# WestlyPark/StyleRenderer

Hardware: AMD Instinct MI355X
Metric: generator fwd+bwd images/sec at 256^2 (higher is better)
Workload: dtype f32

## Files before the change

### include/stylerenderer_amd.h

```cpp
#ifndef STYLERENDERER_AMD_H_
#define STYLERENDERER_AMD_H_

#include <stddef.h>
#include <stdint.h>

#ifdef __cplusplus
extern "C" {
#endif

typedef void* sr_stream_t;

#define SR_OK 0
#define SR_EINVAL (-1)
#define SR_ERANGE (-2)

const char* sr_error_string(int code);
int sr_abi_version(void);

int sr_fused_bias_act(float* y, const float* x, const float* b, const float* ref, int act, int grad,
                      float alpha, float scale, int64_t size_x, int64_t step_b, int64_t size_b,
                      int use_bias, int use_ref, sr_stream_t stream);

int64_t sr_fused_act_bwd_scratch_floats(int64_t n, int64_t c, int64_t inner);
int sr_fused_act_bwd(float* gx, float* gb, const float* gy, const float* out, float alpha,
// ... 258 lines not shown
int sr_conv2d_generic_dgrad(float* dx, const float* g, const float* w, int64_t B, int64_t C, int64_t N, int64_t IH,
                            int64_t IW, int64_t OH, int64_t OW, int kh, int kw, int sy, int sx, int py, int px,
                            sr_stream_t stream);
int sr_conv2d_generic_wgrad(float* dw, const float* x, const float* g, int64_t B, int64_t C, int64_t N, int64_t IH,
                            int64_t IW, int64_t OH, int64_t OW, int kh, int kw, int sy, int sx, int py, int px,
                            sr_stream_t stream);
int sr_conv2d_mfma_ex(float* out, const float* in, const float* wt, const float* iscale,
                      const float* oscale, const float* obias, int64_t B, int64_t C, int64_t N,
                      int64_t wt_ld, int64_t IH, int64_t IW, int64_t OH, int64_t OW, int ksize,
                      int stride, int pad, int transposed, int flags, float* scratch, sr_stream_t stream);
int sr_conv1x1_add_supported(int64_t B, int64_t C, int64_t N, int64_t wt_ld, int64_t P, const float* in, const float* wt,
                             const float* out, const float* addend);
int sr_conv1x1_add(float* out, const float* in, const float* wt, const float* oscale, const float* addend, int64_t B,
                   int64_t C, int64_t N, int64_t wt_ld, int64_t P, sr_stream_t stream);
int sr_conv2d_nba_ex(float* out, const float* in, const float* wt, const float* iscale, const float* oscale,
                     const float* noise, const float* noise_w, const float* abias, float alpha, float gain,
                     int64_t B, int64_t C, int64_t N, int64_t wt_ld, int64_t H, int64_t W, int64_t noise_bstride,
                     int flags, float* scratch, sr_stream_t stream);

int64_t sr_conv2d_wgrad_scratch_floats(int64_t B, int64_t C, int64_t N, int64_t IH, int64_t IW,
                                       int64_t OH, int64_t OW, int ksize, int stride, int pad,
                                       int transposed);
int sr_conv2d_wgrad_mfma(float* dwt, const float* x, const float* gy, const float* xscale,
                         const float* gscale, int64_t B, int64_t C, int64_t N, int64_t IH,
                         int64_t IW, int64_t OH, int64_t OW, int ksize, int stride, int pad,
                         int transposed, float* scratch, sr_stream_t stream);
#define SR_WGRAD_PATH_INVALID (-1)
#define SR_WGRAD_PATH_DIRECT 0
#define SR_WGRAD_PATH_SMALL3 1
#define SR_WGRAD_PATH_WINO 2
#define SR_WGRAD_PATH_BF16_1X1 3
#define SR_WGRAD_PATH_BF16_S2 4
#define SR_WGRAD_PATH_S2_DMA 5
int sr_conv2d_wgrad_path(int64_t B, int64_t C, int64_t N, int64_t IH, int64_t IW, int64_t OH, int64_t OW, int ksize,
                         int stride, int pad, int transposed, const float* x, const float* gy);

int sr_signal_bump(uint32_t* counter, sr_stream_t stream);
int sr_signal_set(uint32_t* word, const uint32_t* epoch, sr_stream_t stream);
int sr_signal_wait(const uint32_t* counter, uint32_t at_least, sr_stream_t stream);
int sr_signal_wait_timeout(const uint32_t* counter, uint32_t at_least, uint64_t timeout_us, int32_t* status_host,
                           int32_t code, sr_stream_t stream);
int sr_signal_wait_poison(const uint32_t* counter, uint32_t at_least, uint64_t timeout_us, int32_t* status_host,
                          int32_t code, float* poison, sr_stream_t stream);
int sr_signal_set_host(uint32_t* word_host, const uint32_t* epoch, sr_stream_t stream);

int sr_graph_replace_memset_nodes(void* hip_graph, int* replaced);
int sr_graph_node_count(void* graph, int* kernel_nodes, int* all_nodes);

int64_t sr_lpips_layer_scratch_floats(int64_t b, int64_t hw);
int sr_lpips_layer_fwd(float* d, const float* f0, const float* t, const float* lin, int64_t b, int64_t c, int64_t hw,
                       int64_t t_bstride, float eps, float* scratch, sr_stream_t stream);
int sr_lpips_layer_bwd(float* gf, const float* gd, const float* f0, const float* t, const float* lin, int64_t b,
                       int64_t c, int64_t hw, int64_t t_bstride, float eps, sr_stream_t stream);
int sr_ppl_endpoints(float* out, const float* a, const float* b, int64_t in_stride, const float* t, int64_t npairs,
                     int64_t d, int mode, int n_ends, float eps, sr_stream_t stream);
int sr_ppl_prep(float* out, const float* img, const float* shift, const float* scale, int64_t n, int64_t h, int64_t w,
                int64_t y0, int64_t x0, int64_t ch, int64_t cw, int64_t oh, int64_t ow, sr_stream_t stream);
int64_t sr_lpips_pair_scratch_floats(int64_t npairs, int64_t n_layers, const int64_t* hw);
int sr_lpips_pair(float* d, const float* const* f, const float* const* lin, const int64_t* c, const int64_t* hw,
                  int64_t n_layers, int64_t npairs, float div, float* scratch, sr_stream_t stream);
int sr_incep_conv(const float* in, const float* wt, const float* bias, int64_t B, int64_t C, int64_t H, int64_t W,
                  int64_t M, int kh, int kw, int stride, int ph, int pw, int nseg, float* const* seg_out,
                  const int64_t* seg_m0, const int64_t* seg_coff, const int64_t* seg_ctot, sr_stream_t stream);
int sr_incep_pool(float* out, const float* in, int64_t B, int64_t C, int64_t H, int64_t W, int mode, int64_t coff,
                  int64_t ctot, sr_stream_t stream);
int sr_incep_gap(float* out, const float* in, int64_t planes, int64_t hw, sr_stream_t stream);
int sr_fstats_update(double* sum, double* gram, double* shift, const float* f, int64_t n, int64_t d, int first,
                     sr_stream_t stream);
// ... 84 lines not shown
```

### stylerenderer_amd/_lib.py

```python
import ctypes
import os

_HERE = os.path.dirname(os.path.abspath(__file__))
LIB_PATH = os.environ.get("STYLERENDERER_AMD_LIB") or os.path.join(_HERE, "libstylerenderer_hip.so")

_i = ctypes.c_int
_l = ctypes.c_int64
_f = ctypes.c_float
_d = ctypes.c_double
_p = ctypes.c_void_p

SIGNATURES = {
    "sr_error_string": (ctypes.c_char_p, [_i]),
    "sr_abi_version": (_i, []),
    "sr_fused_bias_act": (_i, [_p, _p, _p, _p, _i, _i, _f, _f, _l, _l, _l, _i, _i, _p]),
    "sr_fused_act_bwd_scratch_floats": (_l, [_l, _l, _l]),
    "sr_fused_act_bwd": (_i, [_p, _p, _p, _p, _f, _f, _l, _l, _l, _p, _p]),
    "sr_noise_bias_act": (_i, [_p] * 6 + [_f, _f] + [_l] * 4 + [_p]),
    "sr_noise_bias_act_bwd_scratch_floats": (_l, [_l, _l, _l]),
    "sr_noise_bias_act_bwd": (_i, [_p] * 6 + [_f, _f] + [_l] * 4 + [_p, _p]),
    "sr_noise_bias_act_bwd_dot_scratch_floats": (_l, [_l, _l, _l]),
    "sr_noise_bias_act_bwd_dot": (_i, [_p] * 9 + [_f, _f] + [_l] * 4 + [_p, _p]),
    "sr_conv2d_nba": (_i, [_p] * 8 + [_f, _f] + [_l] * 7 + [_p, _p]),
    "sr_conv2d_nba_ex": (_i, [_p] * 8 + [_f, _f] + [_l] * 7 + [_i, _p, _p]),
# ... 55 lines not shown
    "sr_ada_apply": (_i, [_p] * 3 + [_l] * 3 + [_i, _p]),
    "sr_ada_apply_grad": (_i, [_p] * 3 + [_l] * 3 + [_p]),
    "sr_ada_update": (_i, [_p, _p, _d, _d, _p]),
    "sr_upfirdn2d": (_i, [_p, _p, _p, _l] + [_i] * 14 + [_p]),
    "sr_upsample2_add": (_i, [_p] * 4 + [_l] + [_i] * 6 + [_p]),
    "sr_blur_noise_bias_act": (_i, [_p] * 6 + [_f, _f, _l, _l] + [_i] * 6 + [_l, _p]),
    "sr_conv2d_generic": (_i, [_p] * 4 + [_l] * 7 + [_i] * 6 + [_p]),
    "sr_conv2d_generic_dgrad": (_i, [_p] * 3 + [_l] * 7 + [_i] * 6 + [_p]),
    "sr_conv2d_generic_wgrad": (_i, [_p] * 3 + [_l] * 7 + [_i] * 6 + [_p]),
    "sr_blur_nba_bwd_scratch_floats": (_l, [_l, _l, _i, _i]),
    "sr_blur_nba_bwd": (_i, [_p] * 10 + [_f, _f, _l, _l] + [_i] * 5 + [_l, _p, _p]),
    "sr_rasterize_scratch_bytes": (_l, [_l, _l, _l, _l, _i]),
    "sr_rasterize_forward_f32": (_i, [_l] * 5 + [_i] * 3 + [_p] * 5 + [_f, _p, _l, _p, _p, _p, _p, _p]),
    "sr_rasterize_levels_supported": (_i, [_i, _l, _l, _p, _p]),
    "sr_rasterize_forward_levels_f32": (_i, [_i, _l, _l, _l, _p, _p, _i, _i, _i, _p, _p, _f, _p, _l, _p, _p, _p, _p, _p]),
    "sr_rasterize_grad_levels_f32": (_i, [_i, _l, _l, _l, _p, _p, _i, _i, _p, _p, _l] + [_p] * 6 + [_l, _l] + [_p] * 3 + [_f, _p, _p]),
    "sr_rasterize_forward_f64": (_i, [_l] * 5 + [_i] * 3 + [_p] * 5 + [_d, _p, _l, _p, _p, _p, _p, _p]),
    "sr_rasterize_grad_scratch_bytes": (_l, [_l, _l, _l, _i]),
    "sr_rasterize_forward_cpu_f32": (_i, [_l] * 5 + [_i] * 3 + [_p] * 5 + [_f]),
    "sr_rasterize_forward_cpu_f64": (_i, [_l] * 5 + [_i] * 3 + [_p] * 5 + [_d]),
    "sr_rasterize_backward_cpu_f32": (_i, [_l] * 4 + [_i] + [_p] * 3 + [_f]),
    "sr_rasterize_backward_cpu_f64": (_i, [_l] * 4 + [_i] + [_p] * 3 + [_d]),
    "sr_rasterize_backward_f32": (_i, [_l] * 4 + [_i] * 2 + [_p] * 3 + [_f, _p]),
    "sr_rasterize_backward_f64": (_i, [_l] * 4 + [_i] * 2 + [_p] * 3 + [_d, _p]),
    "sr_rasterize_grad_f32": (_i, [_l] * 5 + [_i] * 2 + [_p, _p, _l] + [_p] * 6 + [_l, _l, _p, _p, _p, _f, _p, _p]),
    "sr_conv2d_wgrad_scratch_floats": (_l, [_l] * 7 + [_i] * 4),
    "sr_conv2d_wgrad_mfma": (_i, [_p] * 5 + [_l] * 7 + [_i] * 4 + [_p, _p]),
    "sr_conv2d_scratch_floats": (_l, [_l] * 7 + [_i] * 4),
    "sr_conv2d_mfma": (_i, [_p] * 6 + [_l] * 8 + [_i] * 4 + [_p, _p]),
    "sr_conv2d_uses_winograd": (_i, [_l] * 5 + [_p, _p]),
    "sr_conv2d_path": (_i, [_l] * 7 + [_i] * 4 + [_p, _p, _p, _l, _i]),
    "sr_conv2d_path_floats": (_l, [_l] * 7 + [_i] * 4 + [_p, _p, _p, _l, _i]),
    "sr_conv2d_wgrad_path": (_i, [_l] * 7 + [_i] * 4 + [_p, _p]),
    "sr_conv2d_mfma_ex": (_i, [_p] * 6 + [_l] * 8 + [_i] * 5 + [_p, _p]),
    "sr_conv1x1_add_supported": (_i, [_l] * 5 + [_p] * 4),
    "sr_conv1x1_add": (_i, [_p] * 5 + [_l] * 5 + [_p]),
    "sr_rasterize_grad_f64": (_i, [_l] * 5 + [_i] * 2 + [_p, _p, _l] + [_p] * 6 + [_l, _l, _p, _p, _p, _d, _p, _p]),
    "sr_pose_fwd": (_i, [_p, _p, _p, _p]),
    "sr_pose_bwd": (_i, [_p, _p, _p, _p, _p]),
    "sr_pose_batch_fwd": (_i, [_p, _p, _p, _l, _p]),
    "sr_affine3_fwd": (_i, [_p, _p, _p, _p, _l, _l, _l, _p]),
    "sr_affine3_bwd": (_i, [_p, _p, _p, _p, _l, _l, _l, _p]),
    "sr_morph_fwd": (_i, [_p] * 9 + [_f, _l, _l, _l, _p]),
    "sr_vertex_normals_bwd_f32": (_i, [_p] * 11 + [_l, _l, _l, _f, _p]),
    "sr_morph_gcoeff_scratch_floats": (_l, [_l, _l, _l]),
    "sr_morph_gcoeff": (_i, [_p] * 6 + [_f, _p, _l, _l, _l, _p]),
    "sr_morph_pose_bwd": (_i, [_p] * 5 + [_l, _p]),
    "sr_skin_joints_fwd": (_i, [_p] * 11 + [_f] + [_l] * 4 + [_p]),
    "sr_skin_fwd": (_i, [_p] * 7 + [_l] * 4 + [_p]),
    "sr_skin_bwd_scratch_floats": (_l, [_l, _l, _l]),
    "sr_skin_bwd": (_i, [_p] * 7 + [_l] * 3 + [_p]),
    "sr_skin_joints_bwd": (_i, [_p] * 11 + [_f, _p] + [_l] * 5 + [_p]),
    "sr_blend_z_floats": (_l, [_l, _l, _l]),
    "sr_blend_head": (_i, [_p] * 6 + [_f] + [_l] * 3 + [_p]),
    "sr_blend_fwd": (_i, [_p] * 8 + [_l] * 4 + [_p]),
    "sr_blend_gz": (_i, [_p] * 3 + [_l] * 4 + [_p]),
    "sr_blend_tail": (_i, [_p] * 5 + [_f, _p] + [_l] * 3 + [_p]),
    "sr_resample_u8_scratch_bytes": (_l, [_l] * 6 + [ctypes.POINTER(ctypes.c_int32)] + [_l] * 4),
    "sr_resample_u8": (_i, [_p, _p] + [_l] * 6 + [_p, _p, ctypes.POINTER(ctypes.c_int32), _l] * 2 + [_l] * 4
                       + [_i, _i, _p, _p]),
    "sr_warp_affine_u8": (_i, [_p, _p, _p] + [_l] * 7 + [_i, _i, _i, _p]),
    "sr_landmark_loss_fwd": (_i, [_p] * 8 + [_l] * 5 + [_f, _f, _p]),
    "sr_landmark_loss_bwd": (_i, [_p, _p, _p, _l, _p, _p, _p] + [_l] * 5 + [_i, _p]),
    "sr_landmark_dyn_fwd": (_i, [_p] * 15 + [_l] * 6 + [_i, _f, _f, _l, _l, _f, _f, _p]),
    "sr_landmark_dyn_bwd": (_i, [_p, _p, _p, _l] + [_p] * 7 + [_l] * 6 + [_i, _p]),
    "sr_region_fill": (_i, [_p, _p, _p] + [_l] * 6 + [_p]),
    "sr_region_grow": (_i, [_p, _p, _l, _l, _l, _i, _p]),
    "sr_region_blend_fwd": (_i, [_p] * 6 + [_l] * 4 + [_f] + [_l] * 4 + [_p]),
    "sr_region_blend_bwd": (_i, [_p] * 3 + [_l] * 4 + [_p]),
    "sr_texture_bake": (_i, [_p] * 9 + [_l] * 10 + [_f, _f, _f, _p]),
    "sr_texture_pad": (_i, [_p] * 4 + [_l] * 4 + [_p]),
    "sr_texture_merge": (_i, [_p] * 5 + [_l] * 4 + [_i, _p]),
    "sr_share_rows": (_i, [_p] + [_l] * 3 + [_p]),
    "sr_camera_fwd": (_i, [_p] * 5 + [_l, _l, _p]),
    "sr_camera_bwd": (_i, [_p] * 6 + [_l, _l, _p]),
    "sr_signal_bump": (_i, [_p, _p]),
    "sr_signal_wait": (_i, [_p, ctypes.c_uint32, _p]),
    "sr_signal_set": (_i, [_p, _p, _p]),
    "sr_signal_set_host": (_i, [_p, _p, _p]),
    "sr_signal_wait_timeout": (_i, [_p, ctypes.c_uint32, ctypes.c_uint64, _p, _i, _p]),
    "sr_signal_wait_poison": (_i, [_p, ctypes.c_uint32, ctypes.c_uint64, _p, _i, _p, _p]),
    "sr_graph_replace_memset_nodes": (_i, [_p, ctypes.POINTER(_i)]),
    "sr_graph_node_count": (_i, [_p, ctypes.POINTER(_i), ctypes.POINTER(_i)]),
}

(CONV_PATH_DIRECT, CONV_PATH_WINO, CONV_PATH_S2_BF16, CONV_PATH_S2_WINO, CONV_PATH_GEMM1X1, CONV_PATH_CONVT_TAPS,
 CONV_PATH_CONVT_BF16, CONV_PATH_CONVT_FUSED_KS, CONV_PATH_CONVT_FUSED) = range(9)
CONV_PATH_STRIPS = 0x100
(WGRAD_PATH_DIRECT, WGRAD_PATH_SMALL3, WGRAD_PATH_WINO, WGRAD_PATH_BF16_1X1, WGRAD_PATH_BF16_S2,
 WGRAD_PATH_S2_DMA) = range(6)

_lib = None


class NativeLibraryError(RuntimeError):
    pass


def lib():
    global _lib
    if _lib is not None:
        return _lib
    if not os.path.isfile(LIB_PATH):
        raise NativeLibraryError(
            "stylerenderer_amd: %s not found. Build it with `python -c 'import __graft_entry__ as g; "
            "g.build()'` (hipcc --offload-arch=gfx950). There is no CPU/PyTorch fallback for device "
            "tensors." % LIB_PATH)
    try:
        handle = ctypes.CDLL(LIB_PATH)
    except OSError as e:
        raise NativeLibraryError("stylerenderer_amd: cannot load %s: %s" % (LIB_PATH, e))
    for name, (res, args) in SIGNATURES.items():
        try:
            fn = getattr(handle, name)
        except AttributeError:
            raise NativeLibraryError("stylerenderer_amd: %s does not export %s" % (LIB_PATH, name))
        fn.restype = res
        fn.argtypes = args
    _lib = handle
    return _lib


def check(rc, what=""):
# ... 17 lines not shown
```

### stylerenderer_amd/build.py

```python
import os
import subprocess
import sys

HERE = os.path.dirname(os.path.abspath(__file__))
CSRC = os.path.join(HERE, "csrc")
LIB = os.path.join(HERE, "libstylerenderer_hip.so")
OBJ = os.path.join(HERE, "csrc", "_obj")

ARCH = "gfx950"
COMMON = ["--offload-arch=" + ARCH, "-O3", "-std=c++17", "-fPIC", "-Wno-unused-result",
          "-fhip-fp32-correctly-rounded-divide-sqrt"]
EXACT = ["-ffp-contract=off"]
NOSLP = ["-fno-slp-vectorize"]

SOURCES = [
    ("capi.hip", EXACT),
    ("fused_bias_act.hip", EXACT),
    ("upfirdn2d.hip", EXACT + NOSLP),
    ("rasterize.hip", EXACT),
    ("fused_elem.hip", EXACT),
    ("weight_prep.hip", EXACT),
    ("style_linear.hip", EXACT),
    ("bank_mm.hip", EXACT),
    ("mesh.hip", EXACT),
    ("landmark.hip", EXACT),
    ("region.hip", EXACT),
    ("texture.hip", EXACT),
    ("share.hip", EXACT),
    ("camera.hip", EXACT),
    ("morph.hip", []),
    ("skin.hip", []),
    ("blend.hip", []),
    ("lpips.hip", EXACT),
    ("ppl.hip", EXACT),
    ("augment.hip", EXACT),
    ("resample.hip", EXACT),
    ("warp.hip", EXACT),
    ("conv_mfma.hip", []),
    ("conv_wino.hip", []),
    ("conv_wgrad_wino.hip", []),
    ("conv_wgrad_mfma.hip", []),
    ("conv_wgrad_bf16x3.hip", []),
    ("conv_s2_bf16x3.hip", []),
    ("conv_s2_wino.hip", []),
    ("conv_generic.hip", []),
    ("conv1x1_gemm.hip", []),
    ("inception.hip", []),
]


def _hipcc():
    for c in (os.environ.get("HIPCC"), "/opt/rocm/bin/hipcc", "hipcc"):
        if c and (os.path.isabs(c) and os.path.exists(c) or not os.path.isabs(c)):
            return c
    return "hipcc"


def _deps(src):
    deps = [src, os.path.join(CSRC, "common.h"),
            os.path.join(HERE, "..", "include", "stylerenderer_amd.h"), os.path.abspath(__file__)]
    deps += [os.path.join(CSRC, f) for f in os.listdir(CSRC) if f.endswith(".h")]
    return max(os.path.getmtime(d) for d in deps if os.path.exists(d))


def build_library(force=False, verbose=False):
    os.makedirs(OBJ, exist_ok=True)
    hipcc = _hipcc()
    objs, rebuilt = [], False
    procs = []
    for name, extra in SOURCES:
        src = os.path.join(CSRC, name)
        obj = os.path.join(OBJ, name.replace(".hip", ".o"))
        objs.append(obj)
        if force or not os.path.exists(obj) or os.path.getmtime(obj) < _deps(src):
            cmd = [hipcc] + COMMON + extra + ["-c", src, "-o", obj]
# ... 22 lines not shown
```

### stylerenderer_amd/csrc/conv_wgrad_mfma.hip

```cpp
#include "common.h"
#include "conv_wgrad_bf16x3.h"
#include "conv_wino.h"

#include <algorithm>
#include <cstdlib>

namespace {

typedef float f32x16 __attribute__((ext_vector_type(16)));
typedef const void __attribute__((address_space(1)))* gptr_t;
typedef void __attribute__((address_space(3)))* lptr_t;

__device__ __attribute__((aligned(16))) const float g_wzero_line[4] = {0.f, 0.f, 0.f, 0.f};
__device__ __attribute__((aligned(16))) const float g_wones_line[4] = {1.f, 1.f, 1.f, 1.f};

struct WgradParams {
    const float* U;
    const float* V;
    const float* uscale;
    const float* vscale;
    float* partial;
    int B, CU, CV;
    int UH, UW;
    int GH, GW;
    int dy0, dx0;
    int tiles_x, tiles_y, tiles_b;
    int tiles_u, tiles_v;
    int ks, patches_per_slice;
    int UP, VP;
};

template <int IS, int TY, int TX, int PW, int PH, int PB, int UT, int VT, int NG>
struct WG {
    static constexpr int NWAVE = 4 * NG, THREADS = 256 * NG;
// ... 395 lines not shown
    int pw, ph, pb, ut, vt;
    int tiles_x, tiles_y, tiles_b, tiles_u, tiles_v, ks, pps;
};

Plan make_plan(int is, int B, int CU, int CV, int GH, int GW) {
    Plan pl;
    if (is == 1) {
        if (GW > 16) { pl.pw = 32; pl.ph = 2; pl.pb = 1; }
        else if (GW > 8) { pl.pw = 16; pl.ph = 4; pl.pb = 1; }
        else if (GW > 4) { pl.pw = 8; pl.ph = 8; pl.pb = 1; }
        else { pl.pw = 4; pl.ph = 4; pl.pb = 4; }
        pl.ut = 64; pl.vt = 64;
    } else {
        if (GW > 8) { pl.pw = 16; pl.ph = 4; pl.pb = 1; }
        else { pl.pw = 8; pl.ph = 8; pl.pb = 1; }
        pl.ut = 32; pl.vt = 128;
    }
    pl.tiles_x = (GW + pl.pw - 1) / pl.pw;
    pl.tiles_y = (GH + pl.ph - 1) / pl.ph;
    pl.tiles_b = (B + pl.pb - 1) / pl.pb;
    pl.tiles_u = (CU + pl.ut - 1) / pl.ut;
    pl.tiles_v = (CV + pl.vt - 1) / pl.vt;
    const int npatch = pl.tiles_x * pl.tiles_y * pl.tiles_b;
    const int tiles_uv = pl.tiles_u * pl.tiles_v;
    const int target = (pl.pb == 1 ? 1 : 2) * SR_NUM_CU;
    int ks = (target + tiles_uv - 1) / tiles_uv;
    if (ks > npatch) ks = npatch;
    if (ks < 1) ks = 1;
    pl.pps = (npatch + ks - 1) / ks;
    pl.ks = (npatch + pl.pps - 1) / pl.pps;
    return pl;
}

constexpr int NG_OF(int pb) { return pb == 1 ? 2 : 1; }

template <int IS, int TY, int TX, int PW, int PH, int PB, int UT, int VT>
int launch_wgrad_one(const WgradParams& p, dim3 grid, hipStream_t st) {
    constexpr int NG = NG_OF(PB);
    using G = WG<IS, TY, TX, PW, PH, PB, UT, VT, NG>;
    static_assert(G::LDS_BYTES <= 160 * 1024, "LDS budget");
    auto kern = k_wgrad_mfma<IS, TY, TX, PW, PH, PB, UT, VT, NG>;
    static bool configured = false;
    if (!configured) {
        (void)hipFuncSetAttribute(reinterpret_cast<const void*>(kern),
                                  hipFuncAttributeMaxDynamicSharedMemorySize, G::LDS_BYTES);
        configured = true;
    }
    hipLaunchKernelGGL(kern, grid, dim3(G::THREADS), G::LDS_BYTES, st, p);
    return sr_launch_status();
}

template <int TY, int TX>
int launch_wgrad_s1(const WgradParams& p, const Plan& pl, hipStream_t st) {
    const dim3 grid((unsigned)(pl.tiles_u * pl.tiles_v * pl.ks));
    if (pl.pw == 32) return launch_wgrad_one<1, TY, TX, 32, 2, 1, 64, 64>(p, grid, st);
    if (pl.pw == 16) return launch_wgrad_one<1, TY, TX, 16, 4, 1, 64, 64>(p, grid, st);
    if (pl.pw == 8) return launch_wgrad_one<1, TY, TX, 8, 8, 1, 64, 64>(p, grid, st);
    return launch_wgrad_one<1, TY, TX, 4, 4, 4, 64, 64>(p, grid, st);
}
bool s2_dma_ok(const Plan& pl, int64_t B, int CU, int CV, int UH, int UW, int GH, int GW, int d0) {
    if (sr_env_off("SR_WGRAD_DMA")) return false;
    return pl.pw == 16 && pl.ph == 4 && pl.pb == 1 && pl.ut == 32 && pl.vt == 128 && CU % 32 == 0 && CV % 128 == 0 &&
           GW % 16 == 0 && GH % 4 == 0 && d0 == 0 && UH >= 2 * GH + 1 && UW >= 2 * GW + 1 &&
           B * CU * UH * UW < (1LL << 29) && B * CV * GH * GW < (1LL << 29);
}

// ... 65 lines not shown
        const int j = threadIdx.x;
        partial[((int64_t)blockIdx.x * WS_CM + c) * WS_ROW + j] = (fold[0][j] + fold[1][j]) + (fold[2][j] + fold[3][j]);
    }
}

__global__ __launch_bounds__(4 * WS_ACC) void k_wgrad_small3_finish(float* __restrict__ dwt, const float* __restrict__ partial,
                                                                    int nblk, int C, int N) {
    __shared__ float part[4][WS_ACC];
    const int j = threadIdx.x % WS_ACC, q = threadIdx.x / WS_ACC;
    float a = 0.0f;
#pragma unroll 8
    for (int k = q; k < nblk; k += 4) a += partial[(int64_t)k * WS_ACC + j];
    part[q][j] = a;
    __syncthreads();
    if (q != 0) return;
    const int n = j % WS_NM, t = (j / WS_NM) % 9, c = j / WS_ROW;
    if (c < C && n < N) dwt[((int64_t)t * C + c) * N + n] = (part[0][j] + part[1][j]) + (part[2][j] + part[3][j]);
}

bool wgrad_small_ok(int64_t C, int64_t N, int ksize, int stride, int pad, int transposed) {
    if (sr_env_off("SR_WGRAD_SMALL")) return false;
    return !transposed && ksize == 3 && stride == 1 && pad == 1 && C <= WS_CM && N <= WS_NM;
}

int wgrad_small_blocks(int64_t B, int64_t IH, int64_t IW) {
    const int64_t px = B * IH * IW;
    const int64_t nb = (px + 1023) / 1024;
    return (int)(nb < 1 ? 1 : (nb > 256 ? 256 : nb));
}

struct WgradPlan {
    int path = SR_WGRAD_PATH_INVALID;
    int64_t sized = -1;
    int GH, GW, UH, UW, CU, CV, d0;
    Plan tiles;
};

bool geometry(int64_t B, int64_t C, int64_t N, int64_t IH, int64_t IW, int64_t OH, int64_t OW,
              int ksize, int stride, int pad, int transposed, WgradPlan& w) {
    if (B < 0 || C <= 0 || N <= 0 || IH <= 0 || IW <= 0 || OH <= 0 || OW <= 0) return false;
    if (!(ksize == 3 || ksize == 1) || !(stride == 1 || stride == 2)) return false;
    if (!transposed) {
        if (OH != (IH + 2 * pad - ksize) / stride + 1 || OW != (IW + 2 * pad - ksize) / stride + 1) return false;
        w.GH = (int)OH; w.GW = (int)OW; w.UH = (int)IH; w.UW = (int)IW; w.CU = (int)C; w.CV = (int)N; w.d0 = -pad;
    } else {
        if (ksize != 3 || stride != 2 || pad != 0 || OH != 2 * IH + 1 || OW != 2 * IW + 1) return false;
        w.GH = (int)IH; w.GW = (int)IW; w.UH = (int)OH; w.UW = (int)OW; w.CU = (int)N; w.CV = (int)C; w.d0 = 0;
    }
    return true;
}

WgradPlan make_wgrad_plan(int64_t B, int64_t C, int64_t N, int64_t IH, int64_t IW, int64_t OH, int64_t OW, int ksize,
                          int stride, int pad, int transposed, const void* x, const void* gy) {
    WgradPlan w;
    if (!geometry(B, C, N, IH, IW, OH, OW, ksize, stride, pad, transposed, w)) return w;
    if (wgrad_small_ok(C, N, ksize, stride, pad, transposed)) {
        w.path = SR_WGRAD_PATH_SMALL3;
        w.sized = (int64_t)wgrad_small_blocks(B, IH, IW) * WS_ACC + 4;
        return w;
    }
    const Plan& pl = w.tiles = make_plan(stride, (int)B, w.CU, w.CV, w.GH, w.GW);
    w.path = SR_WGRAD_PATH_DIRECT;
    w.sized = (int64_t)pl.ks * NG_OF(pl.pb) * ksize * ksize * (pl.tiles_u * pl.ut) * (int64_t)(pl.tiles_v * pl.vt) + 4;
    auto candidate = [&](int path, bool take, int64_t floats) {
        w.sized = std::max(w.sized, floats);
        if (take && w.path == SR_WGRAD_PATH_DIRECT) w.path = path;
    };
    if (!transposed && ksize == 3 && stride == 1 && pad == 1 && sr_winograd_enabled() &&
        sr_wgrad_wino_eligible(B, C, N, IH, IW, nullptr, nullptr))
        candidate(SR_WGRAD_PATH_WINO, sr_wgrad_wino_eligible(B, C, N, IH, IW, x, gy),
                  sr_wgrad_wino_scratch_floats(B, C, N, IH, IW));
    if (!transposed && ksize == 1 && stride == 1 && sr_wgrad_bf16x3_enabled('w'))
        candidate(SR_WGRAD_PATH_BF16_1X1, pad == 0 && B > 0 && sr_wgrad_bf16x3_eligible(B, C, N, IH * IW, x, gy),
                  sr_wgrad_bf16x3_scratch_floats(B, C, N, IH * IW));
    if (ksize == 3 && stride == 2 && sr_wgrad_bf16x3_enabled('g'))
        candidate(SR_WGRAD_PATH_BF16_S2,
                  pad == 0 && sr_wgrad_s2_bf16x3_eligible(B, w.CU, w.CV, w.UH, w.UW, w.GH, w.GW, transposed ? x : gy),
                  sr_wgrad_s2_bf16x3_scratch_floats(B, w.CU, w.CV, w.GH, w.GW));
    if (w.path == SR_WGRAD_PATH_DIRECT && ksize == 3 && stride == 2 &&
        s2_dma_ok(pl, B, w.CU, w.CV, w.UH, w.UW, w.GH, w.GW, w.d0))
        w.path = SR_WGRAD_PATH_S2_DMA;
    return w;
}

int reduce_slices(float* dwt, const float* partial, const WgradPlan& w, int ks, int nt, int UP, int VP, int transposed,
                  hipStream_t st) {
    ReduceParams r;
    r.partial = partial; r.out = dwt;
    r.ks = ks; r.nt = nt; r.UP = UP; r.VP = VP; r.CU = w.CU; r.CV = w.CV;
    r.slab = (int64_t)w.CU * w.CV;
    r.su = transposed ? 1 : w.CV;
    r.sv = transposed ? w.CU : 1;
    for (int t = 0; t < 9; ++t) r.tmap[t] = t;
    launch_wgrad_reduce(r, (int64_t)nt * w.CU * w.CV, st);
    return sr_launch_status();
}

}

extern "C" int64_t sr_conv2d_wgrad_scratch_floats(int64_t B, int64_t C, int64_t N, int64_t IH,
                                                  int64_t IW, int64_t OH, int64_t OW, int ksize,
                                                  int stride, int pad, int transposed) {
    return make_wgrad_plan(B, C, N, IH, IW, OH, OW, ksize, stride, pad, transposed, nullptr, nullptr).sized;
}

extern "C" int sr_conv2d_wgrad_path(int64_t B, int64_t C, int64_t N, int64_t IH, int64_t IW, int64_t OH, int64_t OW,
                                    int ksize, int stride, int pad, int transposed, const float* x, const float* gy) {
    return make_wgrad_plan(B, C, N, IH, IW, OH, OW, ksize, stride, pad, transposed, x, gy).path;
}

extern "C" int sr_conv2d_wgrad_mfma(float* dwt, const float* x, const float* gy, const float* xscale,
                                    const float* gscale, int64_t B, int64_t C, int64_t N, int64_t IH,
                                    int64_t IW, int64_t OH, int64_t OW, int ksize, int stride, int pad,
                                    int transposed, float* scratch, sr_stream_t stream) {
    const WgradPlan w = make_wgrad_plan(B, C, N, IH, IW, OH, OW, ksize, stride, pad, transposed, x, gy);
    if (w.path == SR_WGRAD_PATH_INVALID) return SR_EINVAL;
    if (!dwt || !x || !gy || !scratch) return SR_EINVAL;
    if (B * C * IH * IW >= (1LL << 31) || B * N * OH * OW >= (1LL << 31)) return SR_ERANGE;
    hipStream_t st = sr_stream(stream);
    const float *U = transposed ? gy : x, *V = transposed ? x : gy;
    const float *uscale = transposed ? gscale : xscale, *vscale = transposed ? xscale : gscale;
    int ks = 0, UP = 0, VP = 0, rc = SR_OK;
    switch (w.path) {
    case SR_WGRAD_PATH_SMALL3: {
        const int nb = B > 0 ? wgrad_small_blocks(B, IH, IW) : 0;
        if (nb > 0) {
            hipLaunchKernelGGL(k_wgrad_small3, dim3(nb, (unsigned)C), dim3(256), 0, st, scratch, x, gy, xscale, gscale, (int)B, (int)C,
                               (int)N, (int)IH, (int)IW);
        }
        hipLaunchKernelGGL(k_wgrad_small3_finish, dim3(1), dim3(4 * WS_ACC), 0, st, dwt, scratch, nb, (int)C, (int)N);
        return sr_launch_status();
    }
    case SR_WGRAD_PATH_WINO:
        return sr_wgrad_wino_3x3(dwt, x, gy, xscale, gscale, B, C, N, IH, IW, scratch, st);
    case SR_WGRAD_PATH_BF16_1X1:
        rc = sr_wgrad_bf16x3_launch(x, gy, xscale, gscale, scratch, B, C, N, IH * IW, &ks, &UP, &VP, st);
        return rc != SR_OK ? rc : reduce_slices(dwt, scratch, w, ks, 1, UP, VP, transposed, st);
    case SR_WGRAD_PATH_BF16_S2:
        rc = sr_wgrad_s2_bf16x3_launch(U, V, uscale, vscale, scratch, B, w.CU, w.CV, w.UH, w.UW, w.GH, w.GW, &ks, &UP, &VP, st);
        return rc != SR_OK ? rc : reduce_slices(dwt, scratch, w, ks, 9, UP, VP, transposed, st);
    }
    const Plan& pl = w.tiles;
    WgradParams p;
    p.U = U; p.V = V; p.uscale = uscale; p.vscale = vscale;
    p.partial = scratch;
    p.B = (int)B; p.CU = w.CU; p.CV = w.CV; p.UH = w.UH; p.UW = w.UW; p.GH = w.GH; p.GW = w.GW;
    p.dy0 = p.dx0 = w.d0;
    p.tiles_x = pl.tiles_x; p.tiles_y = pl.tiles_y; p.tiles_b = pl.tiles_b;
    p.tiles_u = pl.tiles_u; p.tiles_v = pl.tiles_v; p.ks = pl.ks; p.patches_per_slice = pl.pps;
    p.UP = pl.tiles_u * pl.ut; p.VP = pl.tiles_v * pl.vt;
    if (B > 0) {
        const bool dma = w.path == SR_WGRAD_PATH_S2_DMA;
        if (ksize == 3 && stride == 1) rc = launch_wgrad_s1<3, 3>(p, pl, st);
        else if (ksize == 3 && stride == 2) rc = launch_wgrad_s2<3, 3>(p, pl, dma, st);
        else if (ksize == 1 && stride == 1) rc = launch_wgrad_s1<1, 1>(p, pl, st);
        else rc = launch_wgrad_s2<1, 1>(p, pl, dma, st);
        if (rc != SR_OK) return rc;
    }
    return reduce_slices(dwt, scratch, w, B > 0 ? pl.ks * NG_OF(pl.pb) : 0, ksize * ksize, p.UP, p.VP, transposed, st);
}
```

Baseline: 572.2.

## Add Winograd-style weight-gradient kernel for stride-2 3x3 convolutions

Adds a new wgrad path for stride-2 3x3 convs that splits the stride-2 kernel into phase components and applies a Winograd-like transform. It uses MFMA f32 with a double-buffered LDS pipeline fed by buffer-to-LDS DMA, and sums 16 transformed partial planes into the 9 taps in a finish kernel. The path is chosen only above a work threshold, so smaller shapes keep the existing S2 DMA kernel with bit-exact results. It costs a large LDS footprint, extra scratch, and floating-point rounding that differs from the direct path.

```diff
diff --git a/include/stylerenderer_amd.h b/include/stylerenderer_amd.h
--- a/include/stylerenderer_amd.h
+++ b/include/stylerenderer_amd.h
@@ -314,8 +314,11 @@
 #define SR_WGRAD_PATH_BF16_1X1 3
 #define SR_WGRAD_PATH_BF16_S2 4
 #define SR_WGRAD_PATH_S2_DMA 5
+#define SR_WGRAD_PATH_S2_WINO 6
 int sr_conv2d_wgrad_path(int64_t B, int64_t C, int64_t N, int64_t IH, int64_t IW, int64_t OH, int64_t OW, int ksize,
                          int stride, int pad, int transposed, const float* x, const float* gy);
+int64_t sr_conv2d_wgrad_path_floats(int64_t B, int64_t C, int64_t N, int64_t IH, int64_t IW, int64_t OH, int64_t OW,
+                                    int ksize, int stride, int pad, int transposed, const float* x, const float* gy);
 
 int sr_signal_bump(uint32_t* counter, sr_stream_t stream);
 int sr_signal_set(uint32_t* word, const uint32_t* epoch, sr_stream_t stream);
diff --git a/stylerenderer_amd/_lib.py b/stylerenderer_amd/_lib.py
--- a/stylerenderer_amd/_lib.py
+++ b/stylerenderer_amd/_lib.py
@@ -111,6 +111,7 @@
     "sr_conv2d_path": (_i, [_l] * 7 + [_i] * 4 + [_p, _p, _p, _l, _i]),
     "sr_conv2d_path_floats": (_l, [_l] * 7 + [_i] * 4 + [_p, _p, _p, _l, _i]),
     "sr_conv2d_wgrad_path": (_i, [_l] * 7 + [_i] * 4 + [_p, _p]),
+    "sr_conv2d_wgrad_path_floats": (_l, [_l] * 7 + [_i] * 4 + [_p, _p]),
     "sr_conv2d_mfma_ex": (_i, [_p] * 6 + [_l] * 8 + [_i] * 5 + [_p, _p]),
     "sr_conv1x1_add_supported": (_i, [_l] * 5 + [_p] * 4),
     "sr_conv1x1_add": (_i, [_p] * 5 + [_l] * 5 + [_p]),
@@ -167,7 +168,7 @@
  CONV_PATH_CONVT_BF16, CONV_PATH_CONVT_FUSED_KS, CONV_PATH_CONVT_FUSED) = range(9)
 CONV_PATH_STRIPS = 0x100
 (WGRAD_PATH_DIRECT, WGRAD_PATH_SMALL3, WGRAD_PATH_WINO, WGRAD_PATH_BF16_1X1, WGRAD_PATH_BF16_S2,
- WGRAD_PATH_S2_DMA) = range(6)
+ WGRAD_PATH_S2_DMA, WGRAD_PATH_S2_WINO) = range(7)
 
 _lib = None
 
diff --git a/stylerenderer_amd/build.py b/stylerenderer_amd/build.py
--- a/stylerenderer_amd/build.py
+++ b/stylerenderer_amd/build.py
@@ -41,6 +41,7 @@
     ("conv_wgrad_wino.hip", []),
     ("conv_wgrad_mfma.hip", []),
     ("conv_wgrad_bf16x3.hip", []),
+    ("conv_wgrad_s2_wino.hip", []),
     ("conv_s2_bf16x3.hip", []),
     ("conv_s2_wino.hip", []),
     ("conv_generic.hip", []),
diff --git a/stylerenderer_amd/csrc/conv_wgrad_mfma.hip b/stylerenderer_amd/csrc/conv_wgrad_mfma.hip
--- a/stylerenderer_amd/csrc/conv_wgrad_mfma.hip
+++ b/stylerenderer_amd/csrc/conv_wgrad_mfma.hip
@@ -1,5 +1,6 @@
 #include "common.h"
 #include "conv_wgrad_bf16x3.h"
+#include "conv_wgrad_s2_wino.h"
 #include "conv_wino.h"
 
 #include <algorithm>
@@ -461,6 +462,9 @@
     return pl;
 }
 
+constexpr double SR_WGRAD_S2_WINO_MIN_WORK = 6.0e9;
+static_assert(SR_WGRAD_S2_WINO_MIN_WORK > 3.63e9, "k_wgrad_s2_dma keeps the shapes the tests pin bit for bit");
+
 constexpr int NG_OF(int pb) { return pb == 1 ? 2 : 1; }
 
 template <int IS, int TY, int TX, int PW, int PH, int PB, int UT, int VT>
@@ -592,6 +596,7 @@
 struct WgradPlan {
     int path = SR_WGRAD_PATH_INVALID;
     int64_t sized = -1;
+    int64_t needs = -1;
     int GH, GW, UH, UW, CU, CV, d0;
     Plan tiles;
 };
@@ -616,15 +621,15 @@
     if (!geometry(B, C, N, IH, IW, OH, OW, ksize, stride, pad, transposed, w)) return w;
     if (wgrad_small_ok(C, N, ksize, stride, pad, transposed)) {
         w.path = SR_WGRAD_PATH_SMALL3;
-        w.sized = (int64_t)wgrad_small_blocks(B, IH, IW) * WS_ACC + 4;
+        w.sized = w.needs = (int64_t)wgrad_small_blocks(B, IH, IW) * WS_ACC + 4;
         return w;
     }
     const Plan& pl = w.tiles = make_plan(stride, (int)B, w.CU, w.CV, w.GH, w.GW);
     w.path = SR_WGRAD_PATH_DIRECT;
-    w.sized = (int64_t)pl.ks * NG_OF(pl.pb) * ksize * ksize * (pl.tiles_u * pl.ut) * (int64_t)(pl.tiles_v * pl.vt) + 4;
+    w.sized = w.needs = (int64_t)pl.ks * NG_OF(pl.pb) * ksize * ksize * (pl.tiles_u * pl.ut) * (int64_t)(pl.tiles_v * pl.vt) + 4;
     auto candidate = [&](int path, bool take, int64_t floats) {
         w.sized = std::max(w.sized, floats);
-        if (take && w.path == SR_WGRAD_PATH_DIRECT) w.path = path;
+        if (take && w.path == SR_WGRAD_PATH_DIRECT) { w.path = path; w.needs = floats; }
     };
     if (!transposed && ksize == 3 && stride == 1 && pad == 1 && sr_winograd_enabled() &&
         sr_wgrad_wino_eligible(B, C, N, IH, IW, nullptr, nullptr))
@@ -637,6 +642,13 @@
         candidate(SR_WGRAD_PATH_BF16_S2,
                   pad == 0 && sr_wgrad_s2_bf16x3_eligible(B, w.CU, w.CV, w.UH, w.UW, w.GH, w.GW, transposed ? x : gy),
                   sr_wgrad_s2_bf16x3_scratch_floats(B, w.CU, w.CV, w.GH, w.GW));
+    if (ksize == 3 && stride == 2 && sr_wgrad_s2_wino_eligible(B, w.CU, w.CV, w.UH, w.UW, w.GH, w.GW, w.d0)) {
+        const int sw = sr_env_char("SR_WGRAD_S2_WINO");
+        const double work = 18.0 * (double)B * w.CU * w.CV * w.GH * w.GW;
+        const int64_t floats = sr_wgrad_s2_wino_scratch_floats(pl.ks, w.CU, w.CV);
+        if (floats > w.sized) std::abort();
+        candidate(SR_WGRAD_PATH_S2_WINO, sw != '0' && (sw == 'f' || work >= SR_WGRAD_S2_WINO_MIN_WORK), floats);
+    }
     if (w.path == SR_WGRAD_PATH_DIRECT && ksize == 3 && stride == 2 &&
         s2_dma_ok(pl, B, w.CU, w.CV, w.UH, w.UW, w.GH, w.GW, w.d0))
         w.path = SR_WGRAD_PATH_S2_DMA;
@@ -662,6 +674,12 @@
                                                   int64_t IW, int64_t OH, int64_t OW, int ksize,
                                                   int stride, int pad, int transposed) {
     return make_wgrad_plan(B, C, N, IH, IW, OH, OW, ksize, stride, pad, transposed, nullptr, nullptr).sized;
+}
+
+extern "C" int64_t sr_conv2d_wgrad_path_floats(int64_t B, int64_t C, int64_t N, int64_t IH, int64_t IW, int64_t OH,
+                                               int64_t OW, int ksize, int stride, int pad, int transposed, const float* x,
+                                               const float* gy) {
+    return make_wgrad_plan(B, C, N, IH, IW, OH, OW, ksize, stride, pad, transposed, x, gy).needs;
 }
 
 extern "C" int sr_conv2d_wgrad_path(int64_t B, int64_t C, int64_t N, int64_t IH, int64_t IW, int64_t OH, int64_t OW,
@@ -699,6 +717,12 @@
     case SR_WGRAD_PATH_BF16_S2:
         rc = sr_wgrad_s2_bf16x3_launch(U, V, uscale, vscale, scratch, B, w.CU, w.CV, w.UH, w.UW, w.GH, w.GW, &ks, &UP, &VP, st);
         return rc != SR_OK ? rc : reduce_slices(dwt, scratch, w, ks, 9, UP, VP, transposed, st);
+    case SR_WGRAD_PATH_S2_WINO:
+        rc = sr_wgrad_s2_wino_launch(U, V, uscale, vscale, scratch, B, w.CU, w.CV, w.UH, w.UW, w.GH, w.GW, w.tiles.ks,
+                                     w.tiles.pps, st);
+        return rc != SR_OK ? rc
+                           : sr_wgrad_s2_wino_finish(dwt, scratch, w.tiles.ks, w.CU, w.CV, (int64_t)w.CU * w.CV,
+                                                     transposed ? 1 : w.CV, transposed ? w.CU : 1, st);
     }
     const Plan& pl = w.tiles;
     WgradParams p;
diff --git a/stylerenderer_amd/csrc/conv_wgrad_s2_wino.h b/stylerenderer_amd/csrc/conv_wgrad_s2_wino.h
--- /dev/null
+++ b/stylerenderer_amd/csrc/conv_wgrad_s2_wino.h
@@ -0,0 +1,11 @@
+#pragma once
+#include <hip/hip_runtime.h>
+#include <stdint.h>
+
+bool sr_wgrad_s2_wino_eligible(int64_t B, int64_t CU, int64_t CV, int64_t UH, int64_t UW, int64_t GH, int64_t GW, int d0);
+int64_t sr_wgrad_s2_wino_scratch_floats(int64_t ks, int64_t CU, int64_t CV);
+int sr_wgrad_s2_wino_launch(const float* U, const float* V, const float* uscale, const float* vscale, float* partial,
+                            int64_t B, int64_t CU, int64_t CV, int64_t UH, int64_t UW, int64_t GH, int64_t GW, int ks,
+                            int pps, hipStream_t st);
+int sr_wgrad_s2_wino_finish(float* dwt, const float* partial, int ks, int64_t CU, int64_t CV, int64_t slab, int64_t su,
+                            int64_t sv, hipStream_t st);
diff --git a/stylerenderer_amd/csrc/conv_wgrad_s2_wino.hip b/stylerenderer_amd/csrc/conv_wgrad_s2_wino.hip
--- /dev/null
+++ b/stylerenderer_amd/csrc/conv_wgrad_s2_wino.hip
@@ -0,0 +1,289 @@
+#include "common.h"
+#include "conv_wgrad_s2_wino.h"
+
+namespace {
+
+typedef float f32x16 __attribute__((ext_vector_type(16)));
+typedef void __attribute__((address_space(3)))* lptr_t;
+
+__device__ const float g_s2p_one[1] = {1.f};
+
+struct S2pParams {
+    const float* U;
+    const float* V;
+    const float* uscale;
+    const float* vscale;
+    float* partial;
+    int B, CU, CV, UH, UW, GH, GW;
+    int tiles_x, tiles_y, tiles_u, tiles_v;
+    int pps;
+};
+
+namespace s2p {
+constexpr int RP = 36;
+constexpr int UPL = 5 * RP + 1;
+constexpr int URAW = 32 * UPL;
+constexpr int VPL = 8 * 32 + 1;
+constexpr int VBUF = 16 * VPL;
+constexpr int TP = 25 * 32;
+constexpr int UHAT = 8 * TP;
+constexpr int OFF_V = 2 * URAW;
+constexpr int OFF_UH = OFF_V + 2 * VBUF;
+constexpr int LDS_FLOATS = OFF_UH + 2 * UHAT;
+constexpr int LDS_BYTES = LDS_FLOATS * 4;
+static_assert(LDS_BYTES <= 160 * 1024, "LDS budget");
+__device__ constexpr int slot_of(int i) { return i == 0 ? 0 : i == 1 ? 1 : i == 2 ? 2 : i == 3 ? 1 : 3; }
+__device__ constexpr int vsel_of(int i) { return i < 2 ? 0 : i < 4 ? 1 : 2; }
+}
+
+__global__ __launch_bounds__(256) void k_wgrad_s2p(const S2pParams p) {
+#if __HIP_DEVICE_COMPILE__
+    using namespace s2p;
+    extern __shared__ __attribute__((aligned(16))) float smem[];
+    const int bid = blockIdx.x;
+    const int tile_uv = bid % (p.tiles_u * p.tiles_v);
+    const int slice = bid / (p.tiles_u * p.tiles_v);
+    const int u0 = (tile_uv / p.tiles_v) * 32, v0 = (tile_uv % p.tiles_v) * 128;
+    const int tid = threadIdx.x, lane = tid & 63;
+    const int wave = __builtin_amdgcn_readfirstlane(tid >> 6);
+    const int half = lane >> 5, l31 = lane & 31;
+
+    const int nhp = 2 * p.tiles_x * p.tiles_y * p.B;
+    const int first = slice * p.pps * 2;
+    int last = first + p.pps * 2;
+    if (last > nhp) last = nhp;
+    if (first >= last) return;
+    const int plane_u = p.UH * p.UW, plane_v = p.GH * p.GW;
+    const int tiles_xy = p.tiles_x * p.tiles_y;
+
+    const __amdgpu_buffer_rsrc_t r_u = uniform_rsrc(p.U, p.B * p.CU * plane_u * 4);
+    const __amdgpu_buffer_rsrc_t r_v = uniform_rsrc(p.V, p.B * p.CV * plane_v * 4);
+    const int u_lane_off = ((lane / 9) * p.UW + 4 * (lane % 9)) * 4;
+    const int v_lane_off = ((lane >> 3) * 16 * plane_v + ((lane >> 2) & 1) * p.GW + 4 * (lane & 3)) * 4;
+    const bool u_lane = lane < 45;
+    const float* usc = p.uscale ? p.uscale : g_s2p_one;
+    const float* vsc = p.vscale ? p.vscale : g_s2p_one;
+    const int us_on = p.uscale ? 1 : 0, vs_on = p.vscale ? 1 : 0;
+
+    auto clamp_hp = [&](int hp) { return hp < last ? hp : last - 1; };
+    auto sample_of = [&](int hp) { return (hp >> 1) / tiles_xy; };
+    auto origin_u = [&](int hp) {
+        const int patch = hp >> 1, g = hp & 1;
+        const int tx_i = patch % p.tiles_x, ty_i = (patch / p.tiles_x) % p.tiles_y, b = patch / tiles_xy;
+        return ((b * p.CU + u0) * plane_u + (ty_i * 8 + g * 4) * p.UW + tx_i * 32) * 4;
+    };
+    auto origin_v = [&](int hp) {
+        const int patch = hp >> 1, g = hp & 1;
+        const int tx_i = patch % p.tiles_x, ty_i = (patch / p.tiles_x) % p.tiles_y, b = patch / tiles_xy;
+        return ((b * p.CV + v0) * plane_v + (ty_i * 4 + g * 2) * p.GW + tx_i * 16) * 4;
+    };
+    auto dma_u = [&](int i, int org, float* dst) {
+        const int ch = wave + 4 * i;
+        if (u_lane)
+            __builtin_amdgcn_raw_ptr_buffer_load_lds(r_u, (lptr_t)(dst + ch * UPL), 16, u_lane_off,
+                                                     __builtin_amdgcn_readfirstlane(org + ch * plane_u * 4), 0, 0);
+    };
+    auto dma_v = [&](int i, int org, float* dst) {
+        const int l = wave + 4 * i;
+        __builtin_amdgcn_raw_ptr_buffer_load_lds(r_v, (lptr_t)(dst + l * VPL), 16, v_lane_off,
+                                                 __builtin_amdgcn_readfirstlane(org + l * plane_v * 4), 0, 0);
+    };
+    auto load_us = [&](int hp) { return usc[((int64_t)sample_of(hp) * p.CU + u0 + l31) * us_on]; };
+    auto load_vs = [&](int hp) { return vsc[((int64_t)sample_of(hp) * p.CV + v0 + wave * 32 + l31) * vs_on]; };
+
+    const int xr_base = l31 * UPL + 4 * (tid >> 5);
+    const int xw_base = (tid >> 5) * TP + l31;
+    const int a_base = half * TP + l31;
+    const int b_base = (l31 & 15) * VPL + (2 * wave + (l31 >> 4)) * 32 + 2 * half;
+
+    float raw[25], tr[25];
+    auto xf_read = [&](const float* src, int k) { raw[k] = src[xr_base + (k / 5) * RP + (k % 5)]; };
+    auto xf_row = [&](int x, int q, float s) {
+        if (q == 0) tr[4 * 5 + x] = raw[2 * 5 + x] * s;
+        if (q == 1) tr[0 * 5 + x] = raw[0 * 5 + x] * s - tr[4 * 5 + x];
+        if (q == 2) tr[1 * 5 + x] = raw[1 * 5 + x] * s;
+        if (q == 3) tr[2 * 5 + x] = raw[4 * 5 + x] * s - tr[4 * 5 + x];
+        if (q == 4) tr[3 * 5 + x] = raw[3 * 5 + x] * s;
+    };
+    auto xf_col_store = [&](float* dst, int i, int j) {
+        float v;
+        if (j == 0) v = tr[i * 5 + 0] - tr[i * 5 + 2];
+        else if (j == 1) v = tr[i * 5 + 1];
+        else if (j == 2) v = tr[i * 5 + 4] - tr[i * 5 + 2];
+        else if (j == 3) v = tr[i * 5 + 3];
+        else v = tr[i * 5 + 2];
+        dst[xw_base + (i * 5 + j) * 32] = v;
+    };
+
+    f32x16 acc[16];
+#pragma unroll
+    for (int t = 0; t < 16; ++t)
+#pragma unroll
+        for (int r = 0; r < 16; ++r) acc[t][r] = 0.0f;
+
+    {
+        const int o0 = origin_u(first), o1 = origin_u(clamp_hp(first + 1)), ov = origin_v(first);
+#pragma unroll
+        for (int i = 0; i < 8; ++i) dma_u(i, o0, smem);
+#pragma unroll
+        for (int i = 0; i < 8; ++i) dma_u(i, o1, smem + URAW);
+#pragma unroll
+        for (int i = 0; i < 4; ++i) dma_v(i, ov, smem + OFF_V);
+    }
+    float us_next = load_us(clamp_hp(first + 1));
+    float vs_cur = load_vs(first);
+    {
+        const float us0 = load_us(first);
+        asm volatile("s_waitcnt vmcnt(0)\n\ts_barrier" ::: "memory");
+#pragma unroll
+        for (int k = 0; k < 25; ++k) xf_read(smem, k);
+#pragma unroll
+        for (int k = 0; k < 25; ++k) xf_row(k / 5, k % 5, us0);
+#pragma unroll
+        for (int k = 0; k < 25; ++k) xf_col_store(smem + OFF_UH, k / 5, k % 5);
+    }
+
+    const int count = last - first;
+    for (int n = 0; n < count; ++n) {
+        asm volatile("s_waitcnt vmcnt(0) lgkmcnt(0)\n\ts_barrier" ::: "memory");
+        const int cur = n & 1;
+        const float* uh = smem + OFF_UH + cur * UHAT;
+        const float* vb = smem + OFF_V + cur * VBUF;
+        const float* ur = smem + (cur ^ 1) * URAW;
+        float* uh_o = smem + OFF_UH + (cur ^ 1) * UHAT;
+        float* ur_o = smem + cur * URAW;
+        float* vb_o = smem + OFF_V + (cur ^ 1) * VBUF;
+        const int hp_u = clamp_hp(first + n + 2), hp_v = clamp_hp(first + n + 1);
+        const int org_u = origin_u(hp_u), org_v = origin_v(hp_v);
+        const float us_x = us_next, vs = vs_cur;
+        float us_ld = 1.0f, vs_ld = 1.0f;
+
+        float a[25], vr[4], vh[9], vhn[9];
+        auto fetch_v = [&](int step, int k) { vr[k] = vb[b_base + (k >> 1) * 16 + 4 * step + (k & 1)]; };
+        auto make_vh = [&](float* o, int q) {
+            if (q < 4) o[(q >> 1) * 3 + (q & 1)] = vr[q] * vs;
+            if (q == 4) o[2] = o[0] + o[1];
+            if (q == 5) o[5] = o[3] + o[4];
+            if (q == 6) o[6] = o[0] + o[3];
+            if (q == 7) o[7] = o[1] + o[4];
+            if (q == 8) o[8] = o[6] + o[7];
+        };
+#pragma unroll
+        for (int k = 0; k < 4; ++k) fetch_v(0, k);
+        __builtin_amdgcn_sched_barrier(0);
+#pragma unroll
+        for (int k = 0; k < 25; ++k) a[k] = uh[a_base + k * 32];
+        __builtin_amdgcn_sched_barrier(0);
+#pragma unroll
+        for (int q = 0; q < 9; ++q) make_vh(vh, q);
+        __builtin_amdgcn_sched_barrier(0);
+
+#pragma unroll
+        for (int step = 0; step < 4; ++step) {
+#pragma unroll
+            for (int m = 0; m < 25; ++m) {
+                const int i = m / 5, j = m % 5;
+                const int t = slot_of(i) * 4 + slot_of(j);
+                acc[t] = __builtin_amdgcn_mfma_f32_32x32x2f32(a[m], vh[vsel_of(i) * 3 + vsel_of(j)], acc[t], 0, 0, 0);
+                __builtin_amdgcn_sched_barrier(0);
+                if (step < 3) {
+                    a[m] = uh[a_base + (2 * (step + 1)) * TP + m * 32];
+                    if (m < 4) fetch_v(step + 1, m);
+                    if (m >= 12 && m < 21) make_vh(vhn, m - 12);
+                }
+                if (step == 0) {
+                    if (m < 8) dma_u(m, org_u, ur_o);
+                    else if (m < 12) dma_v(m - 8, org_v, vb_o);
+                    else if (m == 21) us_ld = load_us(hp_u);
+                    else if (m == 22) vs_ld = load_vs(hp_v);
+                }
+                if (step == 1) xf_read(ur, m);
+                if (step == 2) xf_row(m / 5, m % 5, us_x);
+                if (step == 3) xf_col_store(uh_o, i, j);
+                __builtin_amdgcn_sched_barrier(0);
+            }
+            if (step < 3) {
+#pragma unroll
+                for (int q = 0; q < 9; ++q) vh[q] = vhn[q];
+            }
+        }
+        us_next = us_ld;
+        vs_cur = vs_ld;
+    }
+    asm volatile("s_waitcnt vmcnt(0)" ::: "memory");
+
+    float* dst = p.partial + (int64_t)slice * 16 * p.CU * p.CV;
+#pragma unroll
+    for (int t = 0; t < 16; ++t)
+#pragma unroll
+        for (int r = 0; r < 16; ++r) {
+            const int u = u0 + (r & 3) + 8 * (r >> 2) + 4 * half;
+            const int v = v0 + wave * 32 + l31;
+            dst[((int64_t)t * p.CU + u) * p.CV + v] = acc[t][r];
+        }
+#endif
+}
+
+struct S2pFinish {
+    const float* partial;
+    float* out;
+    int ks, CU, CV;
+    int64_t slab, su, sv;
+};
+
+__global__ __launch_bounds__(256) void k_wgrad_s2p_finish(const S2pFinish p) {
+    const int64_t plane = (int64_t)p.CU * p.CV;
+    const int64_t total = 9 * plane;
+    for (int64_t i = (int64_t)blockIdx.x * blockDim.x + threadIdx.x; i < total; i += (int64_t)gridDim.x * blockDim.x) {
+        const int t = (int)(i / plane);
+        const int64_t uv = i - (int64_t)t * plane;
+        const int u = (int)(uv / p.CV), v = (int)(uv % p.CV);
+        const int ky = t / 3, kx = t % 3;
+        const int a0 = ky, a1 = ky == 1 ? -1 : 3, b0 = kx, b1 = kx == 1 ? -1 : 3;
+        const float* src = p.partial + uv;
+        float s00 = 0.f, s01 = 0.f, s10 = 0.f, s11 = 0.f;
+        for (int s = 0; s < p.ks; ++s) {
+            const float* q = src + (int64_t)s * 16 * plane;
+            s00 += q[(a0 * 4 + b0) * plane];
+            if (b1 >= 0) s01 += q[(a0 * 4 + b1) * plane];
+            if (a1 >= 0) s10 += q[(a1 * 4 + b0) * plane];
+            if (a1 >= 0 && b1 >= 0) s11 += q[(a1 * 4 + b1) * plane];
+        }
+        p.out[t * p.slab + u * p.su + v * p.sv] = (s00 + s01) + (s10 + s11);
+    }
+}
+
+}
+
+bool sr_wgrad_s2_wino_eligible(int64_t B, int64_t CU, int64_t CV, int64_t UH, int64_t UW, int64_t GH, int64_t GW, int d0) {
+    return B > 0 && CU % 32 == 0 && CV % 128 == 0 && GW % 16 == 0 && GH % 4 == 0 && d0 == 0 && UH >= 2 * GH + 1 &&
+           UW >= 2 * GW + 1 && B * CU * UH * UW < (1LL << 29) && B * CV * GH * GW < (1LL << 29);
+}
+
+int64_t sr_wgrad_s2_wino_scratch_floats(int64_t ks, int64_t CU, int64_t CV) { return ks * 16 * CU * CV; }
+
+int sr_wgrad_s2_wino_launch(const float* U, const float* V, const float* uscale, const float* vscale, float* partial,
+                            int64_t B, int64_t CU, int64_t CV, int64_t UH, int64_t UW, int64_t GH, int64_t GW, int ks,
+                            int pps, hipStream_t st) {
+    S2pParams p;
+    p.U = U; p.V = V; p.uscale = uscale; p.vscale = vscale; p.partial = partial;
+    p.B = (int)B; p.CU = (int)CU; p.CV = (int)CV; p.UH = (int)UH; p.UW = (int)UW; p.GH = (int)GH; p.GW = (int)GW;
+    p.tiles_x = (int)(GW / 16); p.tiles_y = (int)(GH / 4); p.tiles_u = (int)(CU / 32); p.tiles_v = (int)(CV / 128);
+    p.pps = pps;
+    static bool configured = false;
+    if (!configured) {
+        (void)hipFuncSetAttribute(reinterpret_cast<const void*>(k_wgrad_s2p), hipFuncAttributeMaxDynamicSharedMemorySize,
+                                  s2p::LDS_BYTES);
+        configured = true;
+    }
+    hipLaunchKernelGGL(k_wgrad_s2p, dim3((unsigned)(p.tiles_u * p.tiles_v * ks)), dim3(256), s2p::LDS_BYTES, st, p);
+    return sr_launch_status();
+}
+
+int sr_wgrad_s2_wino_finish(float* dwt, const float* partial, int ks, int64_t CU, int64_t CV, int64_t slab, int64_t su,
+                            int64_t sv, hipStream_t st) {
+    S2pFinish r;
+    r.partial = partial; r.out = dwt; r.ks = ks; r.CU = (int)CU; r.CV = (int)CV; r.slab = slab; r.su = su; r.sv = sv;
+    hipLaunchKernelGGL(k_wgrad_s2p_finish, dim3(sr_stream_grid(9 * CU * CV, 256)), dim3(256), 0, st, r);
+    return sr_launch_status();
+}
```

After: 584.6 (median of 6 runs). 2.2% higher.
